# cboin1996/avddpg

Hardware: AMD Instinct MI355X
Metric: env-steps/sec + DDPG updates/sec, 4096x5-vehicle platoons (higher is better)
Workload: dtype f32-class (fp16 hi+lo operand pairs on the 16-bit matrix cores, f32 accumulate)

## Files before the change

### avddpg_amd/csrc/fset.hip

```cpp
#include "fset_common.h"

namespace avd {
namespace fset {

__device__ __forceinline__ bf16x8 make_xf(float x0, float x1, float x2, float x3, int h) {
    const bf16 a0 = (bf16)x0, a1 = (bf16)x1, a2 = (bf16)x2, a3 = (bf16)x3;
    const bf16 l0 = (bf16)(x0 - (float)a0), l1 = (bf16)(x1 - (float)a1), l2 = (bf16)(x2 - (float)a2), l3 = (bf16)(x3 - (float)a3);
    const bf16 one = (bf16)1.f, zero = (bf16)0.f;
    bf16x8 v;
    v[0] = a0, v[1] = a1, v[2] = a2, v[3] = a3;
    v[4] = h ? one : l0, v[5] = h ? one : l1, v[6] = h ? zero : l2, v[7] = h ? zero : l3;
    return v;
}
__device__ __forceinline__ bf16x8 make_wf(float w0, float w1, float w2, float w3, float b, int h) {
    const bf16 a0 = (bf16)w0, a1 = (bf16)w1, a2 = (bf16)w2, a3 = (bf16)w3, bh = (bf16)b;
    const bf16 l0 = (bf16)(w0 - (float)a0), l1 = (bf16)(w1 - (float)a1), l2 = (bf16)(w2 - (float)a2), l3 = (bf16)(w3 - (float)a3);
    const bf16 bl = (bf16)(b - (float)bh), zero = (bf16)0.f;
    bf16x8 v;
    v[0] = h ? l0 : a0, v[1] = h ? l1 : a1, v[2] = h ? l2 : a2, v[3] = h ? l3 : a3;
    v[4] = h ? bh : a0, v[5] = h ? bl : a1, v[6] = h ? zero : a2, v[7] = h ? zero : a3;
    return v;
}

struct NetP {
// ... 736 lines not shown
    }
    U0 = allsum(U0), U1 = allsum(U1);
#pragma unroll
    for (int k = 0; k < 9; ++k) V[k] = allsum(V[k]);
    if (!have_u) {
        const int oW2 = critic ? L.cW2 : L.aW2, ob2 = critic ? L.cb2 : L.ab2;
        float u0 = 0.f;
        for (int n = jl; n < H2; n += 32) u0 = fmaf(th[oW2 + (long)f * H2 + n], g[ob2 + n], u0);
        U0 = allsum(u0);
        int oW, ob, ff = f, ld = H1, sin = a.S;
        if (!critic) oW = L.aW1, ob = L.ab1;
        else if (f < H1) oW = L.cWs, ob = L.cbs;
        else oW = L.cWa, ob = L.cba, ff = f - H1, ld = HA, sin = 1;
        U1 = th[ob + ff] * V[8];
        for (int k = 0; k < sin; ++k) U1 = fmaf(th[oW + k * ld + ff], V[k] + V[4 + k], U1);
    }
    if (a.bad && *a.bad) U0 = U1 = V[0] = V[4] = V[8] = __uint_as_float(0x7fc00000u);
    if (jl == 0) {
        int og, obe, omm, omv, oW, ob, ff = f, ld = H1, sin = a.S;
        if (!critic) og = L.ag1, obe = L.abe1, omm = L.amm1, omv = L.amv1, oW = L.aW1, ob = L.ab1;
        else if (f < H1) og = L.cgs, obe = L.cbes, omm = L.cmms, omv = L.cmvs, oW = L.cWs, ob = L.cbs;
        else og = L.cga, obe = L.cbea, omm = L.cmma, omv = L.cmva, oW = L.cWa, ob = L.cba, ff = f - H1, ld = HA, sin = 1;
        const float rs1 = 1.0f / sqrtf(st[omv + ff] + BN_EPS), inv1 = rs1 * th[og + ff], mm1 = st[omm + ff];
        g[obe + ff] = U0;
        g[og + ff] = rs1 * (U1 - mm1 * U0);
        g[ob + ff] = inv1 * V[8];
        for (int k = 0; k < sin; ++k) g[oW + k * ld + ff] = inv1 * (V[k] + V[4 + k]);
    }
}
__global__ __launch_bounds__(512) void finalize_small_kernel(const FinArgs a) {
    finalize_small_item(a, blockIdx.x, a.net_lo + blockIdx.y, a.item_base + blockIdx.z * 16 + (threadIdx.x >> 5), threadIdx.x & 31);
}
__device__ __forceinline__ void finalize_w2_row(const FinArgs& a, int f, int set, int net, int n) {
    const bool critic = net;
    const int K = critic ? Critic::K : Actor::K, KG = critic ? Critic::KG : Actor::KG;
    if (f >= K) return;
    const avd_mlp_layout& L = a.L;
    const float* th = a.theta + (long)set * L.theta_size + (critic ? L.actor_size : 0);
    const float* st = a.stats + (long)set * L.stats_size;
    float* g = a.grads + (long)set * L.theta_size + (critic ? L.actor_size : 0);
    int og, obe, omm, omv, ff = f;
    if (!critic) og = L.ag1, obe = L.abe1, omm = L.amm1, omv = L.amv1;
    else if (f < H1) og = L.cgs, obe = L.cbes, omm = L.cmms, omv = L.cmvs;
    else og = L.cga, obe = L.cbea, omm = L.cmma, omv = L.cmva, ff = f - H1;
    const float inv1 = (1.0f / sqrtf(st[omv + ff] + BN_EPS)) * th[og + ff], sh1 = th[obe + ff] - st[omm + ff] * inv1;
    float G = 0.f;
    const float* pg = a.partG[net] + ((long)set * KG + f) * H2 + n;
    const long stride = (long)a.n_sets * KG * H2;
    int j = 0;
    for (; j + 8 <= a.J; j += 8) {
        float v[8];
#pragma unroll
        for (int u = 0; u < 8; ++u) v[u] = pg[(j + u) * stride];
#pragma unroll
        for (int u = 0; u < 8; ++u) G += v[u];
    }
    for (; j < a.J; ++j) G += pg[j * stride];
    const int oW2 = critic ? L.cW2 : L.aW2, ob2 = critic ? L.cb2 : L.ab2;
    if (a.t1_from_g[net]) a.t1p[(((long)net * a.n_sets + set) * Critic::K + f) * H2 + n] = inv1 * th[oW2 + (long)f * H2 + n] * G;
    if (a.c3[net]) G *= a.c3[net][(long)set * VEC + H2 + n];
    if (a.bad && *a.bad) G = __uint_as_float(0x7fc00000u);
    g[oW2 + (long)f * H2 + n] = inv1 * G + sh1 * g[ob2 + n];
}
__global__ __launch_bounds__(128) void finalize_w2_kernel(const FinArgs a) {
    finalize_w2_row(a, blockIdx.x, blockIdx.y, a.net_lo + blockIdx.z, threadIdx.x);
}
__global__ __launch_bounds__(512) void finalize_w2_feat_kernel(const FinArgs a, int n_w2) {
    const int set = blockIdx.y, net = a.net_lo + blockIdx.z, tid = threadIdx.x;
    if ((int)blockIdx.x < n_w2) finalize_w2_row(a, 4 * blockIdx.x + (tid >> 7), set, net, tid & 127);
    else finalize_small_item(a, set, net, H2 + ((int)blockIdx.x - n_w2) * 16 + (tid >> 5), tid & 31);
}
__global__ __launch_bounds__(128) void finalize_t1_kernel(const FinArgs a) {
    const int set = blockIdx.x, net = a.net_lo + blockIdx.y, n = threadIdx.x;
    if (!a.t1_from_g[net]) return;
    const bool critic = net;
    const avd_mlp_layout& L = a.L;
    const float* th = a.theta + (long)set * L.theta_size + (critic ? L.actor_size : 0);
    const float* st = a.stats + (long)set * L.stats_size;
    float* g = a.grads + (long)set * L.theta_size + (critic ? L.actor_size : 0);
    const int K = critic ? Critic::K : Actor::K;
    const int og2 = critic ? L.cg3 : L.ag2, obe2 = critic ? L.cbe3 : L.abe2, omm2 = critic ? L.cmm3 : L.amm2, omv2 = critic ? L.cmv3 : L.amv2;
    const int oW3 = critic ? L.cW3 : L.aW3, ob3 = critic ? L.cb3 : L.ab3;
    const float* tp = a.t1p + ((long)net * a.n_sets + set) * Critic::K * H2 + n;
    float T1 = 0.f;
    int f = 0;
    for (; f + 8 <= K; f += 8) {
        float v[8];
#pragma unroll
        for (int u = 0; u < 8; ++u) v[u] = tp[(long)(f + u) * H2];
#pragma unroll
        for (int u = 0; u < 8; ++u) T1 += v[u];
    }
    for (; f < K; ++f) T1 += tp[(long)f * H2];
    T1 = fmaf(a.c3[net][(long)set * VEC + n], a.s2raw[((long)net * a.n_sets + set) * H2 + n], T1);
    const float D = g[ob3];
    if (a.bad && *a.bad) T1 = __uint_as_float(0x7fc00000u);
    const float rs2 = 1.0f / sqrtf(st[omv2 + n] + BN_EPS), inv2 = rs2 * th[og2 + n], mm2 = st[omm2 + n];
    const float sh2 = th[obe2 + n] - mm2 * inv2, w3 = th[oW3 + n];
    g[oW3 + n] = inv2 * T1 + sh2 * D;
    g[og2 + n] = w3 * rs2 * (T1 - mm2 * D);
}

void launch_finalize(const FinArgs& fa0, hipStream_t st, int net_lo, int n_nets) {
    FinArgs fa = fa0;
    fa.net_lo = net_lo, fa.item_base = 0;
    const int K = (net_lo + n_nets > 1) ? Critic::K : Actor::K;
    if (fa.partU[net_lo]) {
        hipLaunchKernelGGL(finalize_small_kernel, dim3(fa.n_sets, n_nets, (H2 + K + 15) / 16), dim3(512), 0, st, fa);
        hipLaunchKernelGGL(finalize_w2_kernel, dim3(K, fa.n_sets, n_nets), dim3(H2), 0, st, fa);
    } else {
        hipLaunchKernelGGL(finalize_small_kernel, dim3(fa.n_sets, n_nets, H2 / 16), dim3(512), 0, st, fa);
        const int n_w2 = (K + 3) / 4;
        hipLaunchKernelGGL(finalize_w2_feat_kernel, dim3(n_w2 + (K + 15) / 16, fa.n_sets, n_nets), dim3(512), 0, st, fa, n_w2);
    }
    bool any = false;
    for (int net = net_lo; net < net_lo + n_nets; ++net) any = any || fa.t1_from_g[net];
    if (any) hipLaunchKernelGGL(finalize_t1_kernel, dim3(fa.n_sets, n_nets), dim3(H2), 0, st, fa);
}

struct Plan {
    int grid, J;
    size_t W2T[4], W2R[2], vec[4], a2, y, mu, dmu, dz, xfs, xfs2, partH[2], partHs[3], partU[2], partV[2], partG[2], bad, total;
};
int cu_count() {
    static int cache[64] = {0};
    int dev = 0;
    if (hipGetDevice(&dev) != hipSuccess || dev < 0) return 256;
    if (dev < 64 && cache[dev]) return cache[dev];
    hipDeviceProp_t prop;
    if (hipGetDeviceProperties(&prop, dev) != hipSuccess) return 256;
    const int n = prop.multiProcessorCount > 0 ? prop.multiProcessorCount : 256;
    if (dev < 64) cache[dev] = n;
    return n;
}
static Plan make_plan(int n_agents, int n_sets) {
    Plan pl;
    const int P = n_agents / n_sets;
    int J = cu_count() / n_sets;
    if (J < 1) J = 1;
    if (J > P) J = P;
    pl.J = J, pl.grid = J * n_sets;
    size_t o = 0;
    auto take = [&](size_t bytes) {
        const size_t at = o;
        o += (bytes + 255) / 256 * 256;
        return at;
    };
    for (int i = 0; i < 4; ++i) {
        const int KP = (i & 1) ? Critic::KP : Actor::KP, KW = (i & 1) ? Critic::KW : Actor::KW;
        pl.W2T[i] = take(sizeof(bf16) * (size_t)n_sets * H2 * KW);
        pl.vec[i] = take(sizeof(float) * (size_t)n_sets * VEC);
        if (i < 2) pl.W2R[i] = take(sizeof(bf16) * (size_t)n_sets * KP * H2);
    }
    const size_t rows = (size_t)n_agents * TILE;
    pl.a2 = take(4 * rows), pl.y = take(4 * rows), pl.mu = take(4 * rows), pl.dmu = take(4 * rows);
    pl.dz = take(sizeof(bf16) * rows * H2);
    pl.xfs = take(sizeof(bf16) * rows * 16), pl.xfs2 = take(sizeof(bf16) * rows * 16);
    for (int i = 0; i < 2; ++i) {
        const int KP = i ? Critic::KP : Actor::KP, KG = i ? Critic::KG : Actor::KG;
        pl.partH[i] = take(4 * (size_t)pl.grid * 8 * H2);
        pl.partU[i] = take(4 * (size_t)pl.grid * 2 * 2 * KP * 2);
        pl.partV[i] = take(4 * (size_t)pl.grid * 2 * KP * 16);
        pl.partG[i] = take(4 * (size_t)pl.grid * KG * H2);
    }
    for (int i = 0; i < 3; ++i) pl.partHs[i] = take(4 * (size_t)pl.grid * 8 * 2);
    pl.bad = take(sizeof(int));
    pl.total = o;
    return pl;
}
static int check_fset(const avd_mlp_layout* L, int n_agents, int n_sets, const char* who) {
    AVD_REQUIRE(L, "%s: null layout", who);
    if (L->H1 != H1 || L->H2 != H2 || L->Ha != HA || L->A != 1 || (L->S != 3 && L->S != 4) || L->B != TILE) {
        set_error("%s: serves the reference widths only (layer1 256, layer2 128, action layer 48, A = 1, S in {3, 4}, B = 64); "
                  "got H1=%d H2=%d Ha=%d A=%d S=%d B=%d (avd_learn_shared_bf16 takes other widths)",
                  who, L->H1, L->H2, L->Ha, L->A, L->S, L->B);
        return AVD_E_UNSUPPORTED;
    }
    AVD_REQUIRE(n_sets > 0 && n_sets <= 64 && n_agents > 0 && n_agents % n_sets == 0, "%s: n_agents=%d n_sets=%d", who, n_agents,
                n_sets);
    return AVD_OK;
}

template <int S>
// ... 103 lines not shown
```

### avddpg_amd/csrc/fsplit.hip

```cpp
#include <type_traits>

#include "fset_common.h"
#include "anchor.h"
#include "smooth.h"

namespace avd {
namespace fsplit {
using namespace fset;

struct ActorS {
    static constexpr int K = 256, KP = 256, NFT = 8, NKS = 16, LD = 264, NGT = 9, KG = 288;
    static constexpr bool critic = false;
};
struct CriticS {
    static constexpr int K = 304, KP = 320, NFT = 10, NKS = 19, LD = 312, NGT = 10, KG = 320;
    static constexpr bool critic = true;
};
constexpr int NGT_MAX = 10;

template <int I, int N, class F>
__device__ __forceinline__ void static_for(F&& f) {
    if constexpr (I < N) {
        f(std::integral_constant<int, I>{});
        static_for<I + 1, N>(f);
// ... 109 lines not shown
    const bool any = __ballot(hit) != 0;
    if ((threadIdx.x & 63) == 0) wave_flags[threadIdx.x >> 6] = any;
}
template <int S>
__device__ __forceinline__ void pack_x_role(const PackArgs& a, int which, long bx, unsigned* wave_flags) {
    const float* x = a.x[which];
    const float* extra = a.extra[which];
    const bool extra_is_action = which == 0;
    const long i = bx * 256 + threadIdx.x;
    bool nf = false;
    if (i < 2 * a.rows) {
        float v[4];
        load_x<S>(x, i >> 1, v);
        nf = not_finite(v[0]) || not_finite(v[1]) || not_finite(v[2]) || not_finite(v[3]);
        nf = nf || fmaxf(fmaxf(fabsf(v[0]), fabsf(v[1])), fmaxf(fabsf(v[2]), fabsf(v[3]))) >= F16_OVERFLOW;
        if (!(i & 1)) {
            const float e = extra[i >> 1];
            nf = nf || not_finite(e) || (extra_is_action && fabsf(e) >= F16_OVERFLOW);
        }
        a.outh[which][i] = make_xh(v[0], v[1], v[2], v[3], (int)(i & 1));
    }
    front_flag(wave_flags, nf);
}

struct PrepArgs {
    avd_mlp_layout L;
    int S;
    const float *theta, *stats, *theta_t, *stats_t;
    f16 *Whi[4], *Wlo[4];
    f16 *Wchi[4], *Wclo[4];
    f16x8* wf1h[4];
    float* vec[4];
    unsigned* wap;
    unsigned* smax;
    int* bad;
    unsigned* fflag;
    int n_fflag;
};
constexpr int SCALE_SLICES = 16;
__device__ __forceinline__ float pow2_for(float mx) {
    int e = 0;
    if (mx > 0.f && !not_finite(mx)) (void)frexpf(mx, &e);
    int k = 13 - e;
    k = k < -14 ? -14 : (k > 30 ? 30 : k);
    return ldexpf(1.f, k);
}
__device__ __forceinline__ void scale_role(const PrepArgs& a, int net, int set, int slice, int n_sets) {
    __shared__ float red[256], red2[256], c3a[H2], inva[CriticS::K];
    const int tid = threadIdx.x;
    const bool critic = net & 1, target = net >= 2;
    const avd_mlp_layout& L = a.L;
    const float* th = (target ? a.theta_t : a.theta) + (long)set * L.theta_size + (critic ? L.actor_size : 0);
    const float* st = (target ? a.stats_t : a.stats) + (long)set * L.stats_size;
    const int K = critic ? CriticS::K : ActorS::K, oW2 = critic ? L.cW2 : L.aW2;
    const int og2 = critic ? L.cg3 : L.ag2, omv2 = critic ? L.cmv3 : L.amv2, oW3 = critic ? L.cW3 : L.aW3;
    if (tid < H2) c3a[tid] = fabsf((1.0f / sqrtf(st[omv2 + tid] + BN_EPS)) * th[og2 + tid] * th[oW3 + tid]);
    for (int f = tid; f < K; f += 256) {
        int og, omv, ff = f;
        if (!critic) og = L.ag1, omv = L.amv1;
        else if (f < H1) og = L.cgs, omv = L.cmvs;
        else og = L.cga, omv = L.cmva, ff = f - H1;
        inva[f] = fabsf((1.0f / sqrtf(st[omv + ff] + BN_EPS)) * th[og + ff]);
    }
    __syncthreads();
    const int total = K * H2, per = (total + SCALE_SLICES - 1) / SCALE_SLICES, lo = slice * per, hi = min(total, lo + per);
    float m = 0.f, m2 = 0.f;
    for (int i = lo + tid; i < hi; i += 256) {
        const float w = fabsf(th[oW2 + i]);
        m = fmaxf(m, inva[i / H2] * w);
        m2 = fmaxf(m2, c3a[i % H2] * w);
    }
    red[tid] = m, red2[tid] = m2;
    __syncthreads();
    for (int o = 128; o > 0; o >>= 1) {
        if (tid < o) red[tid] = fmaxf(red[tid], red[tid + o]), red2[tid] = fmaxf(red2[tid], red2[tid + o]);
        __syncthreads();
    }
    if (tid == 0) {
        unsigned* dst = a.smax + (((long)net * n_sets + set) * SCALE_SLICES + slice) * 2;
        dst[0] = __float_as_uint(red[0]);
        dst[1] = __float_as_uint(red2[0]);
    }
}
__global__ __launch_bounds__(320) void prep_kernel(const PrepArgs a) {
    __shared__ float red[320];
    const int n = blockIdx.x, net = blockIdx.y, set = blockIdx.z, f = threadIdx.x;
    const bool critic = net & 1, target = net >= 2;
    const avd_mlp_layout& L = a.L;
    const float* th = (target ? a.theta_t : a.theta) + (long)set * L.theta_size + (critic ? L.actor_size : 0);
    const float* st = (target ? a.stats_t : a.stats) + (long)set * L.stats_size;
    const int K = critic ? CriticS::K : ActorS::K, KP = critic ? CriticS::KP : ActorS::KP;
    const int oW2 = critic ? L.cW2 : L.aW2, ob2 = critic ? L.cb2 : L.ab2, oW3 = critic ? L.cW3 : L.aW3, ob3 = critic ? L.cb3 : L.ab3;
    const int og2 = critic ? L.cg3 : L.ag2, obe2 = critic ? L.cbe3 : L.abe2, omm2 = critic ? L.cmm3 : L.amm2, omv2 = critic ? L.cmv3 : L.amv2;
    const float inv2n = (1.0f / sqrtf(st[omv2 + n] + BN_EPS)) * th[og2 + n], c3n = inv2n * th[oW3 + n];
    const unsigned* smax = a.smax + ((long)net * gridDim.z + set) * SCALE_SLICES * 2;
    unsigned mx = 0, mxc = 0;
#pragma unroll
    for (int sl = 0; sl < SCALE_SLICES; ++sl) mx = max(mx, smax[2 * sl]), mxc = max(mxc, smax[2 * sl + 1]);
    const float SW = pow2_for(__uint_as_float(mx)), SWC = pow2_for(__uint_as_float(mxc));
    if (net == 0 && set == 0) {
        unsigned any = 0;
        for (int w0 = n * 320 + f; w0 < a.n_fflag; w0 += 4 * H2 * 320) {
            unsigned v[4];
#pragma unroll
            for (int u = 0; u < 4; ++u) v[u] = a.fflag[min(w0 + u * H2 * 320, a.n_fflag - 1)];
#pragma unroll
            for (int u = 0; u < 4; ++u) any |= w0 + u * H2 * 320 < a.n_fflag ? v[u] : 0u;
        }
        if (any) atomicOr(a.bad, 1);
    }
    float shw = 0.f;
    if (f < KP) {
        float w = 0.f, inv = 0.f;
        if (f < K) {
            int og, obe, omm, omv, ff = f;
            if (!critic) og = L.ag1, obe = L.abe1, omm = L.amm1, omv = L.amv1;
            else if (f < H1) og = L.cgs, obe = L.cbes, omm = L.cmms, omv = L.cmvs;
            else og = L.cga, obe = L.cbea, omm = L.cmma, omv = L.cmva, ff = f - H1;
            inv = (1.0f / sqrtf(st[omv + ff] + BN_EPS)) * th[og + ff];
            const float sh = th[obe + ff] - st[omm + ff] * inv;
            w = th[oW2 + (long)f * H2 + n];
            shw = sh * w;
            if (not_finite(w) || not_finite(inv) || not_finite(sh)) atomicOr(a.bad, 1);
            f16 hi, lo;
            const float ws = SW * (inv * w);
            if (fabsf(ws) >= F16_OVERFLOW) atomicOr(a.bad, 1);
            split1h(ws, hi, lo);
            const long at = ((long)set * H2 + n) * K + wpos(f);
            a.Whi[net][at] = hi, a.Wlo[net][at] = lo;
        }
        if (!target) {
            f16 hi, lo;
            const float wc = SWC * (c3n * w);
            if (fabsf(wc) >= F16_OVERFLOW) atomicOr(a.bad, 1);
            split1h(wc, hi, lo);
            const long at = ((long)set * KP + f) * H2 + n;
            a.Wchi[net][at] = hi, a.Wclo[net][at] = lo;
        }
    }
    red[f] = shw;
    __syncthreads();
    if (f < 64) red[f] += red[f + 256];
    __syncthreads();
    for (int o = 128; o > 0; o >>= 1) {
        if (f < o) red[f] += red[f + o];
        __syncthreads();
    }
    float* vec = a.vec[net] + (long)set * VEC;
    if (f == 0) {
        if (n == 0) vec[2 * H2 + 1] = SW, vec[2 * H2 + 2] = SWC;
        vec[n] = th[ob2 + n] + red[0];
        vec[H2 + n] = c3n;
        if (not_finite(vec[n]) || not_finite(c3n) || not_finite(th[ob3])) atomicOr(a.bad, 1);
    }
    if (n == 0) {
        __syncthreads();
        float v = 0.f;
        if (f < H2) {
            const float inv2 = (1.0f / sqrtf(st[omv2 + f] + BN_EPS)) * th[og2 + f];
            v = (th[obe2 + f] - st[omm2 + f] * inv2) * th[oW3 + f];
        }
        red[f] = v;
        __syncthreads();
        for (int o = 64; o > 0; o >>= 1) {
            if (f < o) red[f] += red[f + o];
            __syncthreads();
        }
        if (f == 0) vec[2 * H2] = th[ob3] + red[0];
    }
}
__device__ __forceinline__ bool prep1_role(const PrepArgs& a, int ft, int net, int set, int lane) {
    const int r = lane & 31, h = lane >> 5;
    bool hit = false;
    const bool critic = net & 1, target = net >= 2;
    const avd_mlp_layout& L = a.L;
    const float* th = (target ? a.theta_t : a.theta) + (long)set * L.theta_size + (critic ? L.actor_size : 0);
    const int K = critic ? CriticS::K : ActorS::K;
    const int f = 32 * ft + r;
    float w[4] = {0.f, 0.f, 0.f, 0.f}, b = 0.f;
    if (f == K) {
        b = 1.f;
    } else if (f < K) {
        if (critic && ft >= 8) {
            w[0] = th[L.cWa + (f - H1)], b = th[L.cba + (f - H1)];
        } else {
            const float* W = th + (critic ? L.cWs : L.aW1);
#pragma unroll
            for (int k = 0; k < 4; ++k) w[k] = k < a.S ? W[k * H1 + f] : 0.f;
            b = th[(critic ? L.cbs : L.ab1) + f];
        }
        if (not_finite(w[0]) || not_finite(w[1]) || not_finite(w[2]) || not_finite(w[3]) || not_finite(b)) hit = true;
        if (S1 * fmaxf(fmaxf(fabsf(w[0]), fabsf(w[1])), fmaxf(fmaxf(fabsf(w[2]), fabsf(w[3])), fabsf(b))) >= F16_OVERFLOW) hit = true;
    }
    a.wf1h[net][((long)set * NGT_MAX + ft) * 64 + lane] = make_wh(w[0], w[1], w[2], w[3], b, S1, h);
    if (net == 1 && ft == 0 && lane < 48) {
        const int hl = lane / 24, hh = (lane / 12) & 1, ks = (lane / 4) % 3, m = lane & 3;
        unsigned v = 0;
#pragma unroll
        for (int e = 0; e < 2; ++e) {
            const int jj = 2 * m + e, fa = 16 * ks + 8 * (jj >> 2) + 4 * hh + (jj & 3);
            f16 hi, lo;
            split1h(S1 * th[L.cWa + fa], hi, lo);
            v |= (unsigned)__builtin_bit_cast(unsigned short, hl ? lo : hi) << (16 * e);
        }
        a.wap[(long)set * 48 + lane] = v;
    }
    return hit;
}

struct FrontArgs {
    PrepArgs pa;
    PackArgs pk;
    float* grads;
    long n_grads;
    int n_sets, n_scale, n_prep1, n_zero, n_pack;
};
constexpr int ZERO_PER_BLOCK = 4096;
template <int S>
__global__ __launch_bounds__(256) void front_kernel(const FrontArgs a) {
    int b = blockIdx.x;
    if (b < a.n_scale) {
        scale_role(a.pa, b & 3, (b >> 2) % a.n_sets, (b >> 2) / a.n_sets, a.n_sets);
        return;
    }
    b -= a.n_scale;
    if (b < a.n_prep1) {
        const int q = 4 * b + (threadIdx.x >> 6);
        bool hit = false;
        if (q < NGT_MAX * 4 * a.n_sets) hit = prep1_role(a.pa, q % NGT_MAX, (q / NGT_MAX) & 3, q / (NGT_MAX * 4), threadIdx.x & 63);
        front_flag(a.pa.fflag + 4 * (long)b, hit);
        return;
    }
    b -= a.n_prep1;
    if (b < a.n_zero) {
        if (b == 0 && threadIdx.x == 0) *a.pa.bad = 0;
        const long base = (long)b * ZERO_PER_BLOCK + threadIdx.x;
#pragma unroll
        for (int k = 0; k < ZERO_PER_BLOCK / 256; ++k)
            if (base + 256 * k < a.n_grads) a.grads[base + 256 * k] = 0.f;
        return;
    }
    b -= a.n_zero;
    const int which = b >= a.n_pack;
    pack_x_role<S>(a.pk, which, b - which * a.n_pack, a.pa.fflag + 4 * ((long)a.n_prep1 + b));
}

enum HeadMode { OUT_TANH = 0, OUT_TD = 1, HEAD_BOTH = 5, OUT_TANH_SAVE = 6, HEAD_CRITIC = 7 };
struct HeadArgs {
    unsigned long long* stamp;
    NetP net;
    int n_agents, n_sets;
// ... 1132 lines not shown
}
#endif
template <int S, class... H>
static int run(int phases, const avd_mlp_layout& L, int n_agents, int n_sets, const float* theta, const float* stats, const float* theta_t,
               const float* stats_t, const float* s, const float* a, const float* r, const float* s2, const float* aw, float gamma,
               float high, float* grads, float* losses, unsigned char* ws, const Plan& pl, hipStream_t st, const AnchorArgs* an,
               const SmoothArgs* smo, H... hp) {
    PrepArgs pa;
    pa.L = L, pa.S = S, pa.theta = theta, pa.stats = stats, pa.theta_t = theta_t, pa.stats_t = stats_t;
    pa.wap = (unsigned*)(ws + pl.wap), pa.bad = (int*)(ws + pl.bad), pa.smax = (unsigned*)(ws + pl.smax);
    pa.fflag = (unsigned*)(ws + pl.fflag), pa.n_fflag = pl.n_fflag;
    NetP net[4];
    for (int i = 0; i < 4; ++i) {
        const bool critic = i & 1, target = i >= 2;
        pa.Whi[i] = (f16*)(ws + pl.Whi[i]), pa.Wlo[i] = (f16*)(ws + pl.Wlo[i]), pa.vec[i] = (float*)(ws + pl.vec[i]);
        pa.wf1h[i] = (f16x8*)(ws + pl.wf1h[i]);
        pa.Wchi[i] = i < 2 ? (f16*)(ws + pl.Wchi[i]) : nullptr, pa.Wclo[i] = i < 2 ? (f16*)(ws + pl.Wclo[i]) : nullptr;
        NetP& n = net[i];
        n.th = (target ? theta_t : theta) + (critic ? L.actor_size : 0), n.th_stride = L.theta_size;
        n.Whi = pa.Whi[i], n.Wlo = pa.Wlo[i], n.Wchi = pa.Wchi[i], n.Wclo = pa.Wclo[i], n.wf1h = pa.wf1h[i], n.vec = pa.vec[i];
        n.wap = pa.wap;
    }
    const int P = n_agents / n_sets;
    const float inv_n = 1.0f / ((float)P * TILE);
    const long nrows = (long)n_agents * TILE;
    f16x8 *xfs = (f16x8*)(ws + pl.xfs), *xfs2 = (f16x8*)(ws + pl.xfs2);
    int* bad = (int*)(ws + pl.bad);
    float *a2 = (float*)(ws + pl.a2), *y = (float*)(ws + pl.y), *mu = (float*)(ws + pl.mu), *dmu = (float*)(ws + pl.dmu);
    float *g3 = (float*)(ws + pl.g3), *g3a = (float*)(ws + pl.g3a);
    unsigned *sm = (unsigned*)(ws + pl.sm), *sma = (unsigned*)(ws + pl.sma);
    auto F = [&](size_t off) { return (float*)(ws + off); };
    const dim3 grid(pl.grid), block(NT);
    HeadArgs h;
    h.n_agents = n_agents, h.n_sets = n_sets, h.gamma = gamma, h.high = high, h.inv_n = inv_n, h.aw = aw, h.sm = sm, h.g3 = g3, h.dmu = dmu;
    h.act2 = nullptr, h.part_s2 = nullptr, h.stamp = nullptr, h.bad = bad, h.part_m = nullptr, h.tz = F(pl.tz), h.abl = 0;
    if (const char* e = AVD_DIAG_ENV("FSPLIT_ABL")) h.abl = atoi(e);
    auto head_args = [&](int ni, const f16x8* x, const float* act, const float* rr, const float* yin, float* out, float* part_s) {
        h.net = net[ni], h.xf = x, h.act = act, h.r = rr, h.yin = yin, h.out = out, h.part_s = part_s;
#ifdef AVD_STAMP
        h.stamp = head_stamps() + 128 * ni;
#endif
        return h;
    };
    auto head = [&](auto kern, int ni, const f16x8* x, const float* act, const float* rr, const float* yin, float* out, float* part_s,
                    auto... extra) {
        hipLaunchKernelGGL(kern, grid, block, 0, st, head_args(ni, x, act, rr, yin, out, part_s), extra...);
    };
    DwArgs dw;
    dw.n_agents = n_agents, dw.n_sets = n_sets, dw.sm = sm, dw.g3 = g3, dw.x = s, dw.stamp = nullptr, dw.abl = 0;
    if (const char* e = AVD_DIAG_ENV("FSPLIT_ABL")) dw.abl = atoi(e);
#ifdef AVD_STAMP
    static unsigned long long* d_stamp = nullptr;
    if (!d_stamp) (void)hipMalloc(&d_stamp, 128 * 8);
    dw.stamp = d_stamp;
#endif
    DxArgs dx;
    dx.n_agents = n_agents, dx.n_sets = n_sets, dx.sm = sm, dx.g3 = g3, dx.xfh = xfs, dx.stamp = nullptr, dx.L_cWa = dx.L_cba = 0;
    dx.abl = dw.abl;
#ifdef AVD_STAMP
    dx.stamp = d_stamp;
#endif
    FinArgs fa;
    fa.L = L, fa.n_sets = n_sets, fa.J = pl.J, fa.S = S, fa.nrh = 1, fa.theta = theta, fa.stats = stats, fa.grads = grads, fa.losses = losses;
    fa.inv_n = inv_n, fa.partLa = F(pl.partHs[2]), fa.bad = bad;
    for (int i = 0; i < 2; ++i)
        fa.partH[i] = nullptr, fa.partHs[i] = F(pl.partHs[i]), fa.partU[i] = nullptr, fa.partV[i] = F(pl.partV[i]),
        fa.partG[i] = F(pl.partG[i]), fa.c3[i] = F(pl.vec[i]);
    fa.t1_from_g[0] = fa.t1_from_g[1] = 1, fa.t1p = F(pl.t1p), fa.s2raw = F(pl.s2raw);
    bool fused = phases == PH_BOTH && !an && !smo && sizeof...(H) == 0;
#ifdef AVD_STAMP
    fused = false;
#endif
    if (AVD_DIAG_ENV("FSPLIT_UNFUSED")) fused = false;
    SeedArgs sd;
    sd.n_agents = n_agents, sd.n_sets = n_sets, sd.dmu = dmu, sd.tz = F(pl.tz), sd.high = high, sd.g3 = g3a, sd.part_m = F(pl.partM[0]),
    sd.part_s = F(pl.partHs[0]);
    if (phases & (PH_CRITIC | PH_TD)) {
        FrontArgs fr;
        fr.pa = pa, fr.grads = grads, fr.n_grads = (long)n_sets * L.theta_size, fr.n_sets = n_sets;
        fr.pk.x[0] = s, fr.pk.extra[0] = a, fr.pk.outh[0] = xfs, fr.pk.x[1] = s2, fr.pk.extra[1] = r, fr.pk.outh[1] = xfs2, fr.pk.rows = nrows;
        fr.n_scale = 4 * n_sets * SCALE_SLICES, fr.n_prep1 = pl.n_prep1, fr.n_pack = pl.n_pack;
        fr.n_zero = (int)((fr.n_grads + ZERO_PER_BLOCK - 1) / ZERO_PER_BLOCK);
        hipLaunchKernelGGL(front_kernel<S>, dim3((unsigned)(fr.n_scale + fr.n_prep1 + fr.n_zero + 2 * fr.n_pack)), dim3(256), 0, st, fr);
        hipLaunchKernelGGL(prep_kernel, dim3(H2, 4, n_sets), dim3(320), 0, st, pa);
    }
    if (fused) {
        FwdArgs fw;
        fw.tanh_t = head_args(2, xfs2, nullptr, nullptr, nullptr, a2, nullptr);
        fw.td = head_args(3, xfs2, a2, r, nullptr, y, nullptr);
        h.sm = sma;
        fw.tanh_save = head_args(0, xfs, nullptr, nullptr, nullptr, mu, nullptr);
        h.sm = sm;
        h.act2 = mu, h.part_s2 = F(pl.partHs[2]), h.part_m = F(pl.partM[1]);
        fw.both = head_args(1, xfs, a, nullptr, y, nullptr, F(pl.partHs[1]));
        fw.seed = sd;
        hipLaunchKernelGGL(forward_kernel<S>, grid, block, 0, st, fw);
        BwdArgs bw;
        dw.net = net[1], dw.act = a, dw.partG = F(pl.partG[1]), dw.part_m = F(pl.partM[1]);
        bw.dw_c = dw;
        dx.net = net[1], dx.partV = F(pl.partV[1]), dx.act = a, dx.part_m = F(pl.partM[1]);
        bw.dx_c = dx;
        dx.L_cWa = L.cWa, dx.L_cba = L.cba;
        bw.dxa = dx;
        dw.sm = sma, dw.g3 = g3a, dw.net = net[0], dw.act = nullptr, dw.partG = F(pl.partG[0]), dw.part_m = F(pl.partM[0]);
        bw.dw_a = dw;
        dx.sm = sma, dx.g3 = g3a, dx.net = net[0], dx.partV = F(pl.partV[0]), dx.act = nullptr, dx.part_m = F(pl.partM[0]), dx.L_cWa = dx.L_cba = 0;
        bw.dx_a = dx;
        hipLaunchKernelGGL(backward_kernel<S>, grid, block, 0, st, bw);
        launch_finalize(fa, st, 0, 2);
        return check_launch("avd_learn_set_split");
    }
    const bool td = phases == PH_TD;
    if (phases & (PH_CRITIC | PH_TD)) {
        head(head_kernel<S, ActorS, OUT_TANH>, 2, xfs2, nullptr, nullptr, nullptr, a2, nullptr);
        if (smo) {
            SmoothArgs q = *smo;
            q.n_agents = n_agents, q.a2 = a2;
            launch_target_smooth(q, st);
        }
        if constexpr (sizeof...(H) > 0)
            head(head_kernel<S, CriticS, OUT_TD, true, H...>, 3, xfs2, a2, r, nullptr, y, nullptr, hp...);
        else
            head(head_kernel<S, CriticS, OUT_TD>, 3, xfs2, a2, r, nullptr, y, nullptr);
        if (!td) {
            h.sm = sma;
            head(head_kernel<S, ActorS, OUT_TANH_SAVE>, 0, xfs, nullptr, nullptr, nullptr, mu, nullptr);
            h.sm = sm;
        }
        h.act2 = td ? nullptr : mu, h.part_s2 = F(pl.partHs[2]), h.part_m = F(pl.partM[1]);
        if (td)
            head(head_kernel<S, CriticS, HEAD_CRITIC>, 1, xfs, a, nullptr, y, nullptr, F(pl.partHs[1]));
        else
            head(head_kernel<S, CriticS, HEAD_BOTH>, 1, xfs, a, nullptr, y, nullptr, F(pl.partHs[1]));
        dw.net = net[1], dw.act = a, dw.partG = F(pl.partG[1]), dw.part_m = F(pl.partM[1]);
        hipLaunchKernelGGL((dw_kernel<S, CriticS>), grid, block, 0, st, dw);
        dx.net = net[1], dx.partV = F(pl.partV[1]), dx.act = a, dx.part_m = F(pl.partM[1]);
        hipLaunchKernelGGL((dx_kernel<S, CriticS>), grid, block, 0, st, dx);
        dx.L_cWa = L.cWa, dx.L_cba = L.cba;
        hipLaunchKernelGGL((dxa_kernel<S>), grid, block, 0, st, dx);
        if (phases == PH_CRITIC || td) launch_finalize(fa, st, 1, 1);
    }
    if (phases & PH_ACTOR) {
        if (an) {
            AnchorArgs q = *an;
            q.n_agents = n_agents, q.n_sets = n_sets, q.S = S, q.J = pl.J, q.dmu = dmu, q.tz = sd.tz, q.high = high, q.g3 = g3a;
            q.part_m = sd.part_m, q.part_s = sd.part_s, q.mu = mu, q.s = s, q.aw = aw, q.inv_n = inv_n, q.c = 2.f * an->weight * inv_n;
            q.bad = bad;
            launch_anchor_seed(q, pl.grid, st);
        } else
            hipLaunchKernelGGL(actor_seed_kernel, grid, block, 0, st, sd);
        dw.sm = sma, dx.sm = sma, dw.g3 = g3a, dx.g3 = g3a;
        dw.net = net[0], dw.act = nullptr, dw.partG = F(pl.partG[0]), dw.part_m = F(pl.partM[0]);
        hipLaunchKernelGGL((dw_kernel<S, ActorS>), grid, block, 0, st, dw);
        dx.net = net[0], dx.partV = F(pl.partV[0]), dx.act = nullptr, dx.part_m = F(pl.partM[0]), dx.L_cWa = dx.L_cba = 0;
        hipLaunchKernelGGL((dx_kernel<S, ActorS>), grid, block, 0, st, dx);
        if (phases == PH_ACTOR) launch_finalize(fa, st, 0, 1);
        else launch_finalize(fa, st, 0, 2);
    }
#ifdef AVD_STAMP
    if (AVD_DIAG_ENV("FSPLIT_STAMPS")) print_head_stamps(st);
#endif
    return check_launch("avd_learn_set_split");
}

}
}

// ... 162 lines not shown
```

Measured before the change: 2.197 million.

## Batch prep_kernel over 8 output columns with shared-memory W2 tile and vector stores

prep_kernel now handles 8 output neurons per block instead of one. It stages the W2 column slab through a padded shared tile so global reads are coalesced, and packs the transposed fp16 hi/lo weights into 16-byte stores. The per-block BN inverse and shift for the K features are computed once instead of once per neuron, the finite-flag scan is spread across all blocks, and atomicOr calls are merged into one per thread. finalize_t1 also gets a wider unrolled load group and hoisted loads. The tradeoffs are more shared memory and registers per block and a longer strided reduction.

```diff
diff --git a/avddpg_amd/csrc/fset.hip b/avddpg_amd/csrc/fset.hip
--- a/avddpg_amd/csrc/fset.hip
+++ b/avddpg_amd/csrc/fset.hip
@@ -842,8 +842,19 @@
     const int og2 = critic ? L.cg3 : L.ag2, obe2 = critic ? L.cbe3 : L.abe2, omm2 = critic ? L.cmm3 : L.amm2, omv2 = critic ? L.cmv3 : L.amv2;
     const int oW3 = critic ? L.cW3 : L.aW3, ob3 = critic ? L.cb3 : L.ab3;
     const float* tp = a.t1p + ((long)net * a.n_sets + set) * Critic::K * H2 + n;
+    const float c3n = a.c3[net][(long)set * VEC + n], s2n = a.s2raw[((long)net * a.n_sets + set) * H2 + n], D = g[ob3];
+    const float mv2 = st[omv2 + n], g2 = th[og2 + n], mm2 = st[omm2 + n], be2 = th[obe2 + n], w3 = th[oW3 + n];
+    const int isbad = a.bad ? *a.bad : 0;
+    constexpr int T1_GRP = 32;
     float T1 = 0.f;
     int f = 0;
+    for (; f + T1_GRP <= K; f += T1_GRP) {
+        float v[T1_GRP];
+#pragma unroll
+        for (int u = 0; u < T1_GRP; ++u) v[u] = tp[(long)(f + u) * H2];
+#pragma unroll
+        for (int u = 0; u < T1_GRP; ++u) T1 += v[u];
+    }
     for (; f + 8 <= K; f += 8) {
         float v[8];
 #pragma unroll
@@ -852,13 +863,12 @@
         for (int u = 0; u < 8; ++u) T1 += v[u];
     }
     for (; f < K; ++f) T1 += tp[(long)f * H2];
-    T1 = fmaf(a.c3[net][(long)set * VEC + n], a.s2raw[((long)net * a.n_sets + set) * H2 + n], T1);
-    const float D = g[ob3];
-    if (a.bad && *a.bad) T1 = __uint_as_float(0x7fc00000u);
-    const float rs2 = 1.0f / sqrtf(st[omv2 + n] + BN_EPS), inv2 = rs2 * th[og2 + n], mm2 = st[omm2 + n];
-    const float sh2 = th[obe2 + n] - mm2 * inv2, w3 = th[oW3 + n];
-    g[oW3 + n] = inv2 * T1 + sh2 * D;
-    g[og2 + n] = w3 * rs2 * (T1 - mm2 * D);
+    T1 = fmaf(c3n, s2n, T1);
+    if (isbad) T1 = __uint_as_float(0x7fc00000u);
+    const float rs2 = 1.0f / sqrtf(mv2 + BN_EPS), inv2 = rs2 * g2;
+    const float sh2 = fmaf(-mm2, inv2, be2);
+    g[oW3 + n] = fmaf(T1, inv2, sh2 * D);
+    g[og2 + n] = (w3 * rs2) * fmaf(-mm2, D, T1);
 }
 
 void launch_finalize(const FinArgs& fa0, hipStream_t st, int net_lo, int n_nets) {
diff --git a/avddpg_amd/csrc/fsplit.hip b/avddpg_amd/csrc/fsplit.hip
--- a/avddpg_amd/csrc/fsplit.hip
+++ b/avddpg_amd/csrc/fsplit.hip
@@ -215,9 +215,12 @@
         dst[1] = __float_as_uint(red2[0]);
     }
 }
-__global__ __launch_bounds__(320) void prep_kernel(const PrepArgs a) {
-    __shared__ float red[320];
-    const int n = blockIdx.x, net = blockIdx.y, set = blockIdx.z, f = threadIdx.x;
+constexpr int PREP_NC = 8, PREP_LD = PREP_NC + 1, PREP_NT = 320;
+static_assert(H2 % PREP_NC == 0 && PREP_NC % 8 == 0 && CriticS::KP <= PREP_NT && PREP_NC <= 64, "prep_kernel's slab");
+__global__ __launch_bounds__(PREP_NT) void prep_kernel(const PrepArgs a) {
+    __shared__ float tile[PREP_NT * PREP_LD];
+    __shared__ float c3s[PREP_NC], d3r[H2];
+    const int n0 = blockIdx.x * PREP_NC, net = blockIdx.y, set = blockIdx.z, f = threadIdx.x;
     const bool critic = net & 1, target = net >= 2;
     const avd_mlp_layout& L = a.L;
     const float* th = (target ? a.theta_t : a.theta) + (long)set * L.theta_size + (critic ? L.actor_size : 0);
@@ -225,81 +228,110 @@
     const int K = critic ? CriticS::K : ActorS::K, KP = critic ? CriticS::KP : ActorS::KP;
     const int oW2 = critic ? L.cW2 : L.aW2, ob2 = critic ? L.cb2 : L.ab2, oW3 = critic ? L.cW3 : L.aW3, ob3 = critic ? L.cb3 : L.ab3;
     const int og2 = critic ? L.cg3 : L.ag2, obe2 = critic ? L.cbe3 : L.abe2, omm2 = critic ? L.cmm3 : L.amm2, omv2 = critic ? L.cmv3 : L.amv2;
-    const float inv2n = (1.0f / sqrtf(st[omv2 + n] + BN_EPS)) * th[og2 + n], c3n = inv2n * th[oW3 + n];
+    {
+        const float* src = th + oW2 + n0;
+#pragma unroll 8
+        for (int i = f; i < K * PREP_NC; i += PREP_NT) tile[(i / PREP_NC) * PREP_LD + (i % PREP_NC)] = src[(long)(i / PREP_NC) * H2 + (i % PREP_NC)];
+    }
+    if (f < PREP_NC) {
+        const int n = n0 + f;
+        const float inv2n = (1.0f / sqrtf(st[omv2 + n] + BN_EPS)) * th[og2 + n];
+        c3s[f] = inv2n * th[oW3 + n];
+    }
     const unsigned* smax = a.smax + ((long)net * gridDim.z + set) * SCALE_SLICES * 2;
     unsigned mx = 0, mxc = 0;
 #pragma unroll
     for (int sl = 0; sl < SCALE_SLICES; ++sl) mx = max(mx, smax[2 * sl]), mxc = max(mxc, smax[2 * sl + 1]);
     const float SW = pow2_for(__uint_as_float(mx)), SWC = pow2_for(__uint_as_float(mxc));
-    if (net == 0 && set == 0) {
+    bool hit = false;
+    {
+        const int nthr = (int)(gridDim.x * gridDim.y * gridDim.z) * PREP_NT;
+        const int g = (int)((blockIdx.z * gridDim.y + blockIdx.y) * gridDim.x + blockIdx.x) * PREP_NT + f;
         unsigned any = 0;
-        for (int w0 = n * 320 + f; w0 < a.n_fflag; w0 += 4 * H2 * 320) {
+        for (long w0 = g; w0 < a.n_fflag; w0 += 4L * nthr) {
             unsigned v[4];
 #pragma unroll
-            for (int u = 0; u < 4; ++u) v[u] = a.fflag[min(w0 + u * H2 * 320, a.n_fflag - 1)];
-#pragma unroll
-            for (int u = 0; u < 4; ++u) any |= w0 + u * H2 * 320 < a.n_fflag ? v[u] : 0u;
-        }
-        if (any) atomicOr(a.bad, 1);
-    }
-    float shw = 0.f;
-    if (f < KP) {
-        float w = 0.f, inv = 0.f;
+            for (int u = 0; u < 4; ++u) v[u] = a.fflag[min(w0 + (long)u * nthr, (long)a.n_fflag - 1)];
+#pragma unroll
+            for (int u = 0; u < 4; ++u) any |= w0 + (long)u * nthr < a.n_fflag ? v[u] : 0u;
+        }
+        hit = any != 0;
+    }
+    float inv = 0.f, sh = 0.f;
+    if (f < K) {
+        int og, obe, omm, omv, ff = f;
+        if (!critic) og = L.ag1, obe = L.abe1, omm = L.amm1, omv = L.amv1;
+        else if (f < H1) og = L.cgs, obe = L.cbes, omm = L.cmms, omv = L.cmvs;
+        else og = L.cga, obe = L.cbea, omm = L.cmma, omv = L.cmva, ff = f - H1;
+        inv = (1.0f / sqrtf(st[omv + ff] + BN_EPS)) * th[og + ff];
+        sh = th[obe + ff] - st[omm + ff] * inv;
+        hit = hit || not_finite(inv) || not_finite(sh);
+    }
+    __syncthreads();
+    float* trow = tile + f * PREP_LD;
+    unsigned chi[PREP_NC / 2], clo[PREP_NC / 2];
+#pragma unroll
+    for (int c = 0; c < PREP_NC; ++c) {
+        const int n = n0 + c;
+        float w = 0.f, shw = 0.f;
         if (f < K) {
-            int og, obe, omm, omv, ff = f;
-            if (!critic) og = L.ag1, obe = L.abe1, omm = L.amm1, omv = L.amv1;
-            else if (f < H1) og = L.cgs, obe = L.cbes, omm = L.cmms, omv = L.cmvs;
-            else og = L.cga, obe = L.cbea, omm = L.cmma, omv = L.cmva, ff = f - H1;
-            inv = (1.0f / sqrtf(st[omv + ff] + BN_EPS)) * th[og + ff];
-            const float sh = th[obe + ff] - st[omm + ff] * inv;
-            w = th[oW2 + (long)f * H2 + n];
+            w = trow[c];
             shw = sh * w;
-            if (not_finite(w) || not_finite(inv) || not_finite(sh)) atomicOr(a.bad, 1);
+            hit = hit || not_finite(w);
             f16 hi, lo;
             const float ws = SW * (inv * w);
-            if (fabsf(ws) >= F16_OVERFLOW) atomicOr(a.bad, 1);
+            hit = hit || fabsf(ws) >= F16_OVERFLOW;
             split1h(ws, hi, lo);
             const long at = ((long)set * H2 + n) * K + wpos(f);
             a.Whi[net][at] = hi, a.Wlo[net][at] = lo;
         }
-        if (!target) {
-            f16 hi, lo;
-            const float wc = SWC * (c3n * w);
-            if (fabsf(wc) >= F16_OVERFLOW) atomicOr(a.bad, 1);
-            split1h(wc, hi, lo);
-            const long at = ((long)set * KP + f) * H2 + n;
-            a.Wchi[net][at] = hi, a.Wclo[net][at] = lo;
-        }
-    }
-    red[f] = shw;
+        trow[c] = shw;
+        f16 hi, lo;
+        const float wc = SWC * (c3s[c] * w);
+        hit = hit || (!target && f < KP && fabsf(wc) >= F16_OVERFLOW);
+        split1h(wc, hi, lo);
+        const unsigned uh = __builtin_bit_cast(unsigned short, hi), ul = __builtin_bit_cast(unsigned short, lo);
+        if (c & 1) chi[c / 2] |= uh << 16, clo[c / 2] |= ul << 16;
+        else chi[c / 2] = uh, clo[c / 2] = ul;
+    }
+    if (!target && f < KP) {
+        const long at = ((long)set * KP + f) * H2 + n0;
+        uint4* dh = (uint4*)(a.Wchi[net] + at);
+        uint4* dl = (uint4*)(a.Wclo[net] + at);
+#pragma unroll
+        for (int q = 0; q < PREP_NC / 8; ++q) {
+            dh[q] = make_uint4(chi[4 * q], chi[4 * q + 1], chi[4 * q + 2], chi[4 * q + 3]);
+            dl[q] = make_uint4(clo[4 * q], clo[4 * q + 1], clo[4 * q + 2], clo[4 * q + 3]);
+        }
+    }
     __syncthreads();
-    if (f < 64) red[f] += red[f + 256];
+    for (int i = f; i < 64 * PREP_NC; i += PREP_NT) tile[(i / PREP_NC) * PREP_LD + (i % PREP_NC)] += tile[(i / PREP_NC + 256) * PREP_LD + (i % PREP_NC)];
     __syncthreads();
     for (int o = 128; o > 0; o >>= 1) {
-        if (f < o) red[f] += red[f + o];
+        for (int i = f; i < o * PREP_NC; i += PREP_NT) tile[(i / PREP_NC) * PREP_LD + (i % PREP_NC)] += tile[(i / PREP_NC + o) * PREP_LD + (i % PREP_NC)];
         __syncthreads();
     }
     float* vec = a.vec[net] + (long)set * VEC;
-    if (f == 0) {
-        if (n == 0) vec[2 * H2 + 1] = SW, vec[2 * H2 + 2] = SWC;
-        vec[n] = th[ob2 + n] + red[0];
+    if (f == 0 && n0 == 0) vec[2 * H2 + 1] = SW, vec[2 * H2 + 2] = SWC;
+    if (f < PREP_NC) {
+        const int n = n0 + f;
+        const float vn = th[ob2 + n] + tile[f], c3n = c3s[f];
+        vec[n] = vn;
         vec[H2 + n] = c3n;
-        if (not_finite(vec[n]) || not_finite(c3n) || not_finite(th[ob3])) atomicOr(a.bad, 1);
-    }
-    if (n == 0) {
-        __syncthreads();
-        float v = 0.f;
+        hit = hit || not_finite(vn) || not_finite(c3n) || not_finite(th[ob3]);
+    }
+    if (hit) atomicOr(a.bad, 1);
+    if (n0 == 0) {
         if (f < H2) {
             const float inv2 = (1.0f / sqrtf(st[omv2 + f] + BN_EPS)) * th[og2 + f];
-            v = (th[obe2 + f] - st[omm2 + f] * inv2) * th[oW3 + f];
-        }
-        red[f] = v;
+            d3r[f] = (th[obe2 + f] - st[omm2 + f] * inv2) * th[oW3 + f];
+        }
         __syncthreads();
         for (int o = 64; o > 0; o >>= 1) {
-            if (f < o) red[f] += red[f + o];
+            if (f < o) d3r[f] += d3r[f + o];
             __syncthreads();
         }
-        if (f == 0) vec[2 * H2] = th[ob3] + red[0];
+        if (f == 0) vec[2 * H2] = th[ob3] + d3r[0];
     }
 }
 __device__ __forceinline__ bool prep1_role(const PrepArgs& a, int ft, int net, int set, int lane) {
@@ -1598,7 +1630,7 @@
         fr.n_scale = 4 * n_sets * SCALE_SLICES, fr.n_prep1 = pl.n_prep1, fr.n_pack = pl.n_pack;
         fr.n_zero = (int)((fr.n_grads + ZERO_PER_BLOCK - 1) / ZERO_PER_BLOCK);
         hipLaunchKernelGGL(front_kernel<S>, dim3((unsigned)(fr.n_scale + fr.n_prep1 + fr.n_zero + 2 * fr.n_pack)), dim3(256), 0, st, fr);
-        hipLaunchKernelGGL(prep_kernel, dim3(H2, 4, n_sets), dim3(320), 0, st, pa);
+        hipLaunchKernelGGL(prep_kernel, dim3(H2 / PREP_NC, 4, n_sets), dim3(PREP_NT), 0, st, pa);
     }
     if (fused) {
         FwdArgs fw;
```

New measurement: 2.213 million (median of 6 runs). Within noise of the previous version (+0.7%).
